# jsdjayanga/kmer-counter

Hardware: NVIDIA B200
Metric: k-mers counted/s at k=31 (higher is better)
Workload: dtype u64

## Files before the change

### kmer-counter_b200/csrc/kc_super.cu

```cuda
#include <math.h>
#include <stdlib.h>

#include "kc_internal.h"
#include "kc_super.cuh"

namespace kc {

namespace {

constexpr uint32_t kNoBin = 0xffffffffu;
constexpr int kSwThreads = 256;
constexpr int kSwMaxSeg = 18;
constexpr int kNb1Max = 1024;
constexpr int kRsBins = 2048;

template <uint32_t X> struct ILog2 { static constexpr uint32_t v = 1 + ILog2<(X >> 1)>::v; };
template <> struct ILog2<1> { static constexpr uint32_t v = 0; };

__host__ __device__ __forceinline__ uint32_t mmer_hash(uint32_t mm) {
    uint32_t h = mm * 0x9E3779B1u;
    h ^= h >> 15;
    h *= 0x85EBCA6Bu;
    return h;
}
__device__ __forceinline__ uint32_t bin_of_min(uint32_t mn, uint32_t n_bins) {
    return __umulhi(mn * 0xC2B2AE35u, n_bins);
}

struct SwScatterParams {
    ExtractParams ep;
    uint32_t m, w, nh, nh_stride, seg_len, segs_per_read, cmax, span;
    uint32_t h_off, bin_off, bits_off;
    uint32_t n_bins, bin_cap;
    uint64_t ovf_cap;
    uint32_t *cursor;
    uint8_t *bins;
    uint8_t *ovf;
    unsigned long long *sc;
};

template <int W, bool CANON>
__global__ void __launch_bounds__(kSwThreads) sw_scatter_kernel(SwScatterParams q) {
    const ExtractParams &p = q.ep;
    extern __shared__ __align__(128) uint8_t smem[];
    const uint32_t stage_bytes = p.stage_bytes;
    uint8_t *stage0 = smem;
    uint64_t *enc = reinterpret_cast<uint64_t *>(smem + p.enc_off);
    uint8_t *enc_b = reinterpret_cast<uint8_t *>(enc);
    const uint32_t enc_row = p.nw + 1;
    uint8_t *bad4 = smem + p.bad_off;
    uint8_t *flag = smem + p.flag_off;
    uint64_t *bars = reinterpret_cast<uint64_t *>(smem + p.bar_off);
    uint32_t *hh = reinterpret_cast<uint32_t *>(smem + q.h_off);
    uint32_t *bid = reinterpret_cast<uint32_t *>(smem + q.bin_off);
    uint32_t *seg_st = reinterpret_cast<uint32_t *>(smem + q.bits_off);
    uint32_t *seg_bd = seg_st + p.tile_reads * q.segs_per_read;
    __shared__ uint32_t s_nstart;
    const uint32_t tid = threadIdx.x, lane = tid & 31;

    if (tid == 0) {
        s_nstart = 0;
        mbar_init(&bars[0], 1);
        mbar_init(&bars[1], 1);
        mbar_fence_init();
    }
    for (uint32_t i = tid; i < p.tile_reads * enc_row; i += kSwThreads) enc[i] = 0;
    for (uint32_t i = tid; i < p.tile_reads; i += kSwThreads) flag[i] = 0;
    __syncthreads();

    auto tile_reads_of = [&](uint32_t t) -> uint32_t {
        uint64_t first = (uint64_t)t * p.tile_reads;
        uint64_t left = p.n_reads - first;
        return left < p.tile_reads ? (uint32_t)left : p.tile_reads;
    };
    auto issue_load = [&](uint32_t t, uint32_t s) {
        uint32_t bytes = tile_reads_of(t) * p.L;
        const uint8_t *src = p.reads + (uint64_t)t * p.tile_reads * p.L;
        uint8_t *dst = stage0 + s * stage_bytes;
        if ((bytes & 15u) == 0) {
            if (tid == 0) {
                asm volatile("fence.proxy.async.shared::cta;" ::: "memory");
                mbar_expect_tx(&bars[s], bytes);
                tma_load_1d(dst, src, bytes, &bars[s]);
            }
        } else {
            for (uint32_t i = tid; i < bytes; i += kSwThreads) dst[i] = src[i];
        }
    };

    uint32_t phase_bits = 0, stage = 0;
    unsigned long long invalid_local = 0, windows_local = 0, records_local = 0;
    const uint32_t mmask = q.m >= 16 ? 0xffffffffu : ((1u << (2 * q.m)) - 1u);
    const uint32_t mshift = 64 - 2 * q.m;
    const uint32_t ng = (q.nh + 7) >> 3;

    uint32_t tile = blockIdx.x;
    if (tile < p.n_tiles) issue_load(tile, 0);

    for (; tile < p.n_tiles; tile += gridDim.x) {
        const uint32_t next = tile + gridDim.x;
        if (next < p.n_tiles) issue_load(next, stage ^ 1);
        const uint32_t nreads = tile_reads_of(tile);
        if (((nreads * p.L) & 15u) == 0) {
            mbar_wait(&bars[stage], (phase_bits >> stage) & 1u);
            phase_bits ^= 1u << stage;
        } else {
            __syncthreads();
        }
        const uint8_t *src_tile = stage0 + stage * stage_bytes;

        encode_tile(p, src_tile, nreads, enc_b, bad4, flag);
        __syncthreads();
        if (tid == 0) s_nstart = 0;

        for (uint32_t g = tid; g < nreads * ng; g += kSwThreads) {
            const uint32_t r = g / ng, j0 = (g - r * ng) * 8;
            const uint32_t wi = j0 >> 5, sh = (j0 & 31u) * 2u;
            const uint64_t *e = enc + r * enc_row;
            const uint64_t a = wi <= p.nw ? e[wi] : 0ull;
            const uint64_t b = wi + 1 <= p.nw ? e[wi + 1] : 0ull;
            const uint64_t x = sh ? ((a << sh) | (b >> (64 - sh))) : a;
            uint32_t *row = hh + r * q.nh_stride + j0;
            if constexpr (CANON) {
#pragma unroll
                for (uint32_t i = 0; i < 8; i++) {
                    const uint32_t mm = (uint32_t)(x >> (mshift - 2 * i)) & mmask;
                    uint32_t r = __brev(mm);
                    r = ((r >> 1) & 0x55555555u) | ((r & 0x55555555u) << 1);
                    if (j0 + i < q.nh) row[i] = mmer_hash(min(mm, (r >> (32 - 2 * q.m)) ^ mmask));
                }
            } else {
#pragma unroll
                for (uint32_t i = 0; i < 8; i++)
                    if (j0 + i < q.nh) row[i] = mmer_hash((uint32_t)(x >> (mshift - 2 * i)) & mmask);
            }
        }
        __syncthreads();

        const uint32_t n_seg = nreads * q.segs_per_read;
        for (uint32_t sg = tid; sg < n_seg; sg += kSwThreads) {
            const uint32_t r = sg / q.segs_per_read;
            const uint32_t p0 = (sg - r * q.segs_per_read) * q.seg_len;
            if (p0 >= p.nk) { seg_st[sg] = 0; seg_bd[sg] = 0; continue; }
            const uint32_t s = min(q.seg_len, p.nk - p0);
            const uint32_t lb = p0 > 0 ? 1u : 0u;
            const uint32_t se = s + lb;
            const uint32_t *g = hh + r * q.nh_stride + p0 - lb;
            uint32_t S[kSwMaxSeg];
            S[kSwMaxSeg - 1] = 0xffffffffu;
#pragma unroll
            for (int i = kSwMaxSeg - 2; i >= 0; i--) {
                const uint32_t v = (uint32_t)i + 1 < se ? g[i] : 0xffffffffu;
                S[i] = min(v, S[i + 1]);
            }
            uint32_t core = 0xffffffffu;
            for (uint32_t t = se - 1; t < q.w; t++) core = min(core, g[t]);
            uint32_t pm = 0xffffffffu;
            const bool check = flag[r] != 0;
            uint32_t *brow = bid + r * p.nk + p0 - lb;
            uint32_t prev = kNoBin, stm = 0, bdm = 0;
#pragma unroll
            for (uint32_t i = 0; i < (uint32_t)kSwMaxSeg; i++) {
                if (i < se) {
                    const uint32_t mn = min(min(S[i], core), pm);
                    const bool valid = check ? kmer_window_valid(bad4 + r * p.nb4, p0 - lb + i, p.k) : true;
                    const uint32_t b = valid ? bin_of_min(mn, q.n_bins) : kNoBin;
                    if (i >= lb) {
                        if (!valid) invalid_local++;
                        brow[i] = b;
                        const uint32_t st = (valid && b != prev) ? 1u : 0u;
                        stm |= st << (i - lb);
                        bdm |= (st | (valid ? 0u : 1u)) << (i - lb);
                    }
                    prev = b;
                    if (i + 1 < se) pm = min(pm, g[q.w + i]);
                }
            }
            seg_st[sg] = stm;
            seg_bd[sg] = bdm;
        }
        __syncthreads();

        uint32_t *list = hh;
        for (uint32_t base = 0; base < n_seg; base += kSwThreads) {
            const uint32_t sg = base + tid;
            uint32_t stm = sg < n_seg ? seg_st[sg] : 0u;
            const uint32_t cnt = __popc(stm);
            uint32_t incl = cnt;
#pragma unroll
            for (int o = 1; o < 32; o <<= 1) {
                const uint32_t t = __shfl_up_sync(0xffffffffu, incl, o);
                if (lane >= (uint32_t)o) incl += t;
            }
            uint32_t off = 0;
            if (lane == 31 && incl) off = atomicAdd(&s_nstart, incl);
            off = __shfl_sync(0xffffffffu, off, 31) + incl - cnt;
            while (stm) {
                const uint32_t i = __ffs(stm) - 1;
                stm &= stm - 1;
                list[off++] = (sg << 5) | i;
            }
        }
        __syncthreads();
        const uint32_t n_start = s_nstart;
        for (uint32_t en = tid; en < n_start; en += kSwThreads) {
            const uint32_t ent = list[en];
            const uint32_t sg = ent >> 5, wi0 = ent & 31u;
            const uint32_t r = sg / q.segs_per_read, si = sg - r * q.segs_per_read;
            const uint32_t pos = si * q.seg_len + wi0;
            uint32_t end = p.nk;
            {
                uint32_t mk = seg_bd[sg] & ~(0xffffffffu >> (31 - wi0));
                uint32_t sj = si;
                while (mk == 0 && ++sj < q.segs_per_read) mk = seg_bd[r * q.segs_per_read + sj];
                if (mk) end = min(p.nk, sj * q.seg_len + (uint32_t)__ffs(mk) - 1);
            }
            const uint32_t len = end - pos;
            const uint32_t b = bid[r * p.nk + pos];
            const uint64_t *e = enc + r * enc_row;
            for (uint32_t q0 = 0; q0 < len; q0 += q.cmax) {
                const uint32_t idx = atomicAdd(&q.cursor[b], 1u);
                const uint32_t c = min(q.cmax, len - q0);
                const uint32_t wi = (pos + q0) >> 5, sh = ((pos + q0) & 31u) * 2u;
                uint64_t ew[2 * W + 1];
#pragma unroll
                for (int t = 0; t < 2 * W + 1; t++) ew[t] = wi + t <= p.nw ? e[wi + t] : 0ull;
                uint64_t rec[2 * W];
#pragma unroll
                for (int t = 0; t < 2 * W; t++) rec[t] = sh ? ((ew[t] << sh) | (ew[t + 1] >> (64 - sh))) : ew[t];
                const uint32_t nbases = q.span + c - 1;
#pragma unroll
                for (int t = 0; t < 2 * W; t++) {
                    const int keep = (int)nbases - 32 * t;
                    if (keep <= 0) rec[t] = 0;
                    else if (keep < 32) rec[t] &= ~0ull << (64 - 2 * keep);
                }
                rec[2 * W - 1] = (rec[2 * W - 1] & ~0xffull) | c;
                ulonglong2 *dst = nullptr;
                if (idx < q.bin_cap) {
                    dst = reinterpret_cast<ulonglong2 *>(q.bins) + ((uint64_t)b * q.bin_cap + idx) * W;
                } else {
                    const unsigned long long oi = atomicAdd(&q.sc[SW_OVF], 1ull);
                    if (oi < q.ovf_cap) dst = reinterpret_cast<ulonglong2 *>(q.ovf) + oi * W;
                    else atomicOr(&q.sc[SW_FAIL], 1ull);
                }
                if (dst) {
#pragma unroll
                    for (int t = 0; t < W; t++) dst[t] = make_ulonglong2(rec[2 * t], rec[2 * t + 1]);
                }
                windows_local += c;
                records_local++;
            }
        }
        for (uint32_t i = tid; i < nreads; i += kSwThreads) flag[i] = 0;
        __syncthreads();
        stage ^= 1;
    }
#pragma unroll
    for (int o = 16; o > 0; o >>= 1) {
        invalid_local += __shfl_xor_sync(0xffffffffu, invalid_local, o);
        windows_local += __shfl_xor_sync(0xffffffffu, windows_local, o);
        records_local += __shfl_xor_sync(0xffffffffu, records_local, o);
    }
    if (lane == 0) {
        if (invalid_local) atomicAdd(&q.sc[SW_INVALID], invalid_local);
        if (windows_local) atomicAdd(&q.sc[SW_WINDOWS], windows_local);
        if (records_local) atomicAdd(&q.sc[SW_RECORDS], records_local);
    }
}

template <int W> __device__ __forceinline__ bool key_all_ones(const Key<W> &k) {
    uint64_t a = ~0ull;
#pragma unroll
    for (int i = 0; i < W; i++) a &= k.w[i];
    return a == ~0ull;
}
template <int W> __device__ __forceinline__ bool key_any_word_ones(const Key<W> &k) {
    bool r = false;
#pragma unroll
    for (int i = 0; i < W; i++) r = r || (k.w[i] == ~0ull);
    return r;
}
template <int W> __device__ __forceinline__ void key_set_ones(Key<W> &k) {
#pragma unroll
    for (int i = 0; i < W; i++) k.w[i] = ~0ull;
}
__device__ __forceinline__ Key<1> slot_claim(Key<1> *slot, const Key<1> &k) {
    Key<1> o;
    o.w[0] = atomicCAS(reinterpret_cast<unsigned long long *>(slot), ~0ull, (unsigned long long)k.w[0]);
    return o;
}
__device__ __forceinline__ Key<2> slot_claim(Key<2> *slot, const Key<2> &k) {
    Key<2> o;
    const uint32_t a = smem_u32(slot);
    asm volatile(
        "{\n"
        ".reg .b128 c, n, o;\n"
        "mov.b128 c, {%3, %3};\n"
        "mov.b128 n, {%4, %5};\n"
        "atom.shared.cas.b128 o, [%2], c, n;\n"
        "mov.b128 {%0, %1}, o;\n"
        "}\n"
        : "=l"(o.w[0]), "=l"(o.w[1])
        : "r"(a), "l"(~0ull), "l"(k.w[0]), "l"(k.w[1])
        : "memory");
    return o;
}
template <int W> __device__ __forceinline__ uint32_t key_hash(const Key<W> &k) {
    uint32_t x = (uint32_t)k.w[0] ^ (uint32_t)(k.w[0] >> 29);
    if constexpr (W > 1) x ^= ((uint32_t)k.w[W - 1] ^ (uint32_t)(k.w[W - 1] >> 31)) * 0x85EBCA6Bu;
    return x * 0x9E3779B1u;
}
__device__ __forceinline__ uint32_t pass_hash(uint32_t h) { return (h ^ (h >> 15)) * 0x2C1B3C6Du; }

enum {
    SWP_UNIT = 0,
    SWP_DEDUP,
    SWP_SCAN,
    SWP_OPEN,
    SWP_INSERT,
    SWP_DRAIN,
    SWP_ROUND_END,
    SWP_EMIT,
    SWP_PHASES,
    SWP_QUEUED = SWP_PHASES,
    SWP_DRAIN_PROBES,
    SWP_WARPS,
    SWP_TOTAL,
    SWP_SLOTS
};
#ifdef KC_SW_PROFILE
__device__ unsigned long long g_sw_prof[SWP_SLOTS];
#define SWP_DECL                                                                                      \
    __shared__ unsigned long long s_prof[THREADS / 32][SWP_SLOTS];                                    \
    if (lane == 0)                                                                                    \
        for (int i_ = 0; i_ < SWP_SLOTS; i_++) s_prof[warp][i_] = 0;                                  \
    const long long swp_t0 = clock64();                                                               \
    long long swp_t = swp_t0
#define SWP_MARK(ph)                                                                                  \
    do {                                                                                              \
        const long long t_ = clock64();                                                               \
        if (lane == 0) s_prof[warp][ph] += (unsigned long long)(t_ - swp_t);                          \
        swp_t = t_;                                                                                   \
    } while (0)
#define SWP_ADD(c, v) atomicAdd(&s_prof[warp][c], (unsigned long long)(v))
#define SWP_ADD_ACTIVE(c)                                                                             \
    do {                                                                                              \
        const uint32_t am_ = __activemask();                                                          \
        if (lane == (uint32_t)__ffs(am_) - 1) SWP_ADD(c, __popc(am_));                                \
    } while (0)
#define SWP_FLUSH()                                                                                   \
    do {                                                                                              \
        __syncwarp();                                                                                 \
        if (lane == 0) {                                                                              \
            s_prof[warp][SWP_WARPS] = 1;                                                              \
            s_prof[warp][SWP_TOTAL] = (unsigned long long)(clock64() - swp_t0);                       \
            for (int i_ = 0; i_ < SWP_SLOTS; i_++) atomicAdd(&g_sw_prof[i_], s_prof[warp][i_]);       \
        }                                                                                             \
    } while (0)
#else
#define SWP_DECL do {} while (0)
#define SWP_MARK(ph) do {} while (0)
#define SWP_ADD(c, v) do {} while (0)
#define SWP_ADD_ACTIVE(c) do {} while (0)
#define SWP_FLUSH() do {} while (0)
#endif

struct SwCountParams {
    uint32_t n_src;
    const uint32_t *src_cursor[8];
    const uint8_t *src_bins[8];
    const unsigned long long *src_sc[8];
    uint32_t bin_begin;
    const uint8_t *ovf;
    uint32_t n_bins, bin_cap, ovf_slice;
    uint64_t ovf_cap;
    uint64_t last_mask;
    uint64_t *d_keys;
    uint32_t *d_counts;
    uint64_t d_cap;
    uint32_t *hist1;
    int shift1, nb1;
    int add_phantom;
    unsigned long long *sc;
};

template <int W> struct SwCountCfg {
    static constexpr int THREADS = 512, TSLOTS = 4096, RPT = W == 1 ? 2 : 1;
};

template <int W, int THREADS, int TSLOTS, int RPT, bool CANON>
__global__ void __launch_bounds__(THREADS) sw_count_kernel(SwCountParams p) {
    constexpr int RB = THREADS * RPT;
    extern __shared__ __align__(16) uint8_t cs_smem[];
    Key<W> *tk = reinterpret_cast<Key<W> *>(cs_smem);
    ulonglong2 *recs = reinterpret_cast<ulonglong2 *>(tk + TSLOTS);
    uint32_t *tc = reinterpret_cast<uint32_t *>(recs + RB * W);
    uint32_t *s_start = tc + TSLOTS;
    uint32_t *s_hist = s_start + THREADS;
    constexpr int kQueue = RPT > 1 ? 64 : 96;
    Key<W> *queue = reinterpret_cast<Key<W> *>(s_hist + kNb1Max);
    uint32_t *queue_m = reinterpret_cast<uint32_t *>(queue + (THREADS / 32) * kQueue);
    constexpr bool DEDUP = (W == 1);
    constexpr int RT = DEDUP ? RB : 1;
    ulonglong2 *rt_keys = reinterpret_cast<ulonglong2 *>(queue_m + (THREADS / 32) * kQueue);
    uint32_t *rt_mult = reinterpret_cast<uint32_t *>(rt_keys + RT);
    uint32_t *rec_mult = rt_mult + RT;
    __shared__ uint32_t s_unit, s_m, s_ones, s_abort;
    __shared__ unsigned long long s_base;
    __shared__ uint32_t s_warp[THREADS / 32];
// ... 1268 lines not shown
    pl.w = pl.span - pl.m + 1;
    pl.nh = pl.nk + pl.w - 1;
    pl.nh_stride = (pl.nh + 8) | 1u;
    pl.seg_len = pl.w - 1 < (uint32_t)kSwMaxSeg - 1 ? pl.w - 1 : (uint32_t)kSwMaxSeg - 1;
    pl.segs_per_read = (pl.nk + pl.seg_len - 1) / pl.seg_len;
    pl.seg_len = (pl.nk + pl.segs_per_read - 1) / pl.segs_per_read;
}
}

bool super_plan(uint32_t k, uint32_t L, uint32_t flags, uint64_t max_windows, uint32_t occ_per_bin, SuperPlan *out,
                double record_headroom, uint64_t distinct_hint, bool ext_e) {
    if (k == 0 || k > 64 || L < k || L > 4096) return false;
    if (flags & kPlanCanonical) flags |= kPlanStrict;
    const bool strict = (flags & kPlanStrict) != 0;
    SuperPlan pl{};
    pl.flags = flags & (kPlanStrict | kPlanCanonical);
    pl.W = (int)((k + 31) / 32);
    pl.k = k;
    pl.L = L;
    const uint32_t mm = k % 32;
    const bool masked = strict ? (mm != 0) : (mm >= 1 && mm <= 28);
    pl.span = masked ? k : 32u * pl.W;
    pl.last_mask = masked ? (~0ull << (64 - 2 * mm)) : ~0ull;
    if (pl.span < 22) return false;
    pl.nk = L - k + 1;
    pl.cmax = 32u * pl.W - 3;
    if (max_windows == 0) max_windows = 1;
    if (occ_per_bin == 0) {
        occ_per_bin = 8192;
        if (distinct_hint && distinct_hint < max_windows) {
            const double per_key = (double)max_windows / (double)distinct_hint;
            const double occ = 2200.0 * per_key;
            if (occ < 8192.0) occ_per_bin = occ < 1024.0 ? 1024u : ((uint32_t)occ + 255u) & ~255u;
        }
    }
    uint64_t nb = (max_windows + occ_per_bin - 1) / occ_per_bin;
    if (nb < 8) nb = 8;
    if (nb > (1ull << 24)) nb = 1ull << 24;
    pl.n_bins = (uint32_t)nb;
    ExtractParams ep;
    if (!extract_plan(nullptr, 16, L, k, pl.flags, nullptr, &ep, kS1TileBytes)) return false;
    set_minimizer(pl, 12);
    if (s1_smem(pl, ep).total > kS1MaxSmem) return false;
    while (pl.m < 16 && pl.m + 8 < pl.span && (1ull << (2 * pl.m)) < 192ull * pl.n_bins) {
        SuperPlan longer = pl;
        set_minimizer(longer, pl.m + 1);
        if (s1_smem(longer, ep).total > kS1MaxSmem) break;
        pl = longer;
    }
    const double rho = 2.0 / (pl.w + 1) + 1.2 / pl.nk + 1.0 / pl.cmax * 0.25;
    const double est_total = (double)max_windows * rho;
    const double per_bin = est_total / (double)pl.n_bins;
    pl.bin_cap = (uint32_t)(per_bin * (1.0 + 90.0 / sqrt((double)occ_per_bin))) + 64;
    pl.bin_cap = (pl.bin_cap + 3) & ~3u;
    pl.ovf_cap = (uint64_t)(est_total * 0.6) + 8192;
    if (pl.ovf_cap < max_windows / 16) pl.ovf_cap = max_windows / 16;
    pl.ovf_slice = 4096;
    const uint64_t d_base = distinct_hint && distinct_hint < max_windows ? distinct_hint + distinct_hint / 8 + 4096 : max_windows;
    pl.d_cap = d_base + (uint64_t)((double)d_base * record_headroom) + (record_headroom > 0 ? 8192 : 0);
    if (pl.d_cap > (1ull << 32) - 2) pl.d_cap = (1ull << 32) - 2;
    if (pl.d_cap < 1024) pl.d_cap = 1024;
    pl.fin_cap = pl.d_cap > (uint64_t)kSuperMaxSub * (kFinCapSmall * 7 / 10) ? kFinCapLarge : kFinCapSmall;
    pl.sub_target = pl.fin_cap * 7 / 10;
    if (const char *v = getenv("KC_SW_SUB_TARGET")) {
        const int t = atoi(v);
        if (t > 0) pl.sub_target = (uint32_t)t;
    }
    const int sig = pl.W == 1 ? (masked ? (int)(2 * mm) : 64) : 64;
    pl.b1 = sig < 10 ? sig : 10;
    plan_layout(pl, ext_e);
    *out = pl;
    return true;
}

static void plan_layout(SuperPlan &pl, bool ext_e) {
    uint64_t o = 0;
    auto take = [&](uint64_t bytes) { uint64_t r = o; o += round512(bytes); return r; };
    const uint64_t rec_bytes = 16ull * pl.W;
    pl.off_cursor = take((uint64_t)pl.n_bins * 4);
    pl.off_hist1 = take((kNb1Max + 8) * 4);
    pl.off_hist2 = take((uint64_t)(2 * kSuperMaxSub + 8) * 4);
    pl.off_base1 = take((kNb1Max + 8) * 4);
    pl.off_cur1 = take((kNb1Max + 8) * 4);
    pl.off_base2 = take((uint64_t)(kSuperMaxSub + 8) * 4);
    pl.off_cur2 = take((uint64_t)(kSuperMaxSub + 8) * 4);
    pl.off_mout = take((uint64_t)(kSuperMaxSub + 8) * 4);
    pl.off_off = take((uint64_t)(kSuperMaxSub + 8) * 4);
    pl.off_plan = take(sizeof(SuperPlanDev));
    pl.off_x = take(sizeof(XDev));
    pl.off_sc = take(SW_COUNT * 8);
    pl.off_h2m = take((uint64_t)(kSuperMaxSub + 8) * 4);
    pl.off_big = take((uint64_t)(kSuperMaxSub + 8) * 4);
    pl.off_bigoff = take((uint64_t)(kSuperMaxSub + 8) * 4);
    pl.off_bins = take((uint64_t)pl.n_bins * pl.bin_cap * rec_bytes);
    pl.off_ovf = take(pl.ovf_cap * rec_bytes);
    pl.off_dk = take(pl.d_cap * 8 * pl.W + 64);
    pl.off_dc = take(pl.d_cap * 4 + 64);
    pl.ext_e = ext_e;
    pl.ext_ek = nullptr;
    pl.ext_ec = nullptr;
    pl.off_ek = pl.off_ec = o;
    if (!ext_e) {
        pl.off_ek = take(pl.d_cap * 8 * pl.W + 64);
        pl.off_ec = take(pl.d_cap * 4 + 64);
    }
    pl.ws_bytes = o;
}

bool place_plan(uint32_t k, bool strict, uint64_t n_records, SuperPlan *out) {
    if (k == 0 || k > 128 || n_records == 0 || n_records > (1ull << 32) - 2) return false;
    SuperPlan pl{};
    pl.W = (int)((k + 31) / 32);
    pl.k = k;
    const uint32_t mm = k % 32;
    const bool masked = strict ? (mm != 0) : (mm >= 1 && mm <= 28);
    pl.span = masked ? k : 32u * pl.W;
    pl.last_mask = masked ? (~0ull << (64 - 2 * mm)) : ~0ull;
    pl.n_bins = 8;
    pl.d_cap = n_records < 1024 ? 1024 : n_records;
    pl.fin_cap = pl.W >= 3 && n_records <= (uint64_t)kSuperMaxSub * (kFinCapWide * 7 / 10) ? kFinCapWide : kFinCapSmall;
    pl.sub_target = pl.fin_cap * 7 / 10;
    if (const char *v = getenv("KC_SW_SUB_TARGET")) {
        const int t = atoi(v);
        if (t > 0) pl.sub_target = (uint32_t)t;
    }
    const int sig = pl.W == 1 ? (masked ? (int)(2 * mm) : 64) : 64;
    pl.b1 = sig < 10 ? sig : 10;
    plan_layout(pl, false);
    *out = pl;
    return true;
}

namespace {
template <class T> T *at(void *ws, uint64_t off) { return reinterpret_cast<T *>(static_cast<uint8_t *>(ws) + off); }
uint64_t *ek_of(const SuperPlan &pl, void *ws) { return pl.ext_e ? pl.ext_ek : at<uint64_t>(ws, pl.off_ek); }
uint32_t *ec_of(const SuperPlan &pl, void *ws) { return pl.ext_e ? pl.ext_ec : at<uint32_t>(ws, pl.off_ec); }
}

cudaError_t super_reset(const SuperPlan &pl, void *ws, unsigned long long *d_sc, cudaStream_t s) {
    cudaError_t e;
    if ((e = cudaMemsetAsync(ws, 0, pl.off_base1, s)) != cudaSuccess) return e;
    return cudaMemsetAsync(d_sc, 0, SW_COUNT * 8, s);
}

template <int W>
static cudaError_t super_scatter_w(const SuperPlan &pl, const void *d_reads, uint64_t n_reads, void *ws,
                                   unsigned long long *d_sc, int n_sms, cudaStream_t s) {
    SwScatterParams q{};
    if (!extract_plan(d_reads, n_reads, pl.L, pl.k, pl.flags, &d_sc[SW_INVALID], &q.ep, kS1TileBytes))
        return cudaErrorInvalidValue;
    if (q.ep.n_tiles == 0) return cudaSuccess;
    q.m = pl.m; q.w = pl.w; q.nh = pl.nh; q.nh_stride = pl.nh_stride;
    q.seg_len = pl.seg_len; q.segs_per_read = pl.segs_per_read; q.cmax = pl.cmax; q.span = pl.span;
    const S1Smem lay = s1_smem(pl, q.ep);
    q.h_off = lay.h_off;
    q.bin_off = lay.bin_off;
    q.bits_off = lay.bits_off;
    const uint32_t smem = lay.total;
    if (smem > kS1MaxSmem) return cudaErrorInvalidValue;
    q.n_bins = pl.n_bins; q.bin_cap = pl.bin_cap; q.ovf_cap = pl.ovf_cap;
    q.cursor = at<uint32_t>(ws, pl.off_cursor);
    q.bins = at<uint8_t>(ws, pl.off_bins);
    q.ovf = at<uint8_t>(ws, pl.off_ovf);
    q.sc = d_sc;
    auto kern = (pl.flags & kPlanCanonical) ? sw_scatter_kernel<W, true> : sw_scatter_kernel<W, false>;
    cudaError_t e = cudaFuncSetAttribute(kern, cudaFuncAttributeMaxDynamicSharedMemorySize, (int)smem);
    if (e != cudaSuccess) return e;
    int per_sm = 1;
    cudaOccupancyMaxActiveBlocksPerMultiprocessor(&per_sm, kern, kSwThreads, smem);
    per_sm = per_sm < 1 ? 1 : (per_sm > 6 ? 6 : per_sm);
    uint32_t grid = (uint32_t)n_sms * per_sm;
    if (grid > q.ep.n_tiles) grid = q.ep.n_tiles;
    kern<<<grid, kSwThreads, smem, s>>>(q);
    return cudaGetLastError();
}

cudaError_t super_scatter(const SuperPlan &pl, const void *d_reads, uint64_t n_reads, void *ws,
                          unsigned long long *d_sc, int n_sms, cudaStream_t s) {
    if (pl.W == 1) return super_scatter_w<1>(pl, d_reads, n_reads, ws, d_sc, n_sms, s);
    if (pl.W == 2) return super_scatter_w<2>(pl, d_reads, n_reads, ws, d_sc, n_sms, s);
    return cudaErrorInvalidValue;
}

template <int W, bool CANON>
static cudaError_t launch_count(const SwCountParams &cp, int n_sms, cudaStream_t s) {
    constexpr uint32_t THREADS = SwCountCfg<W>::THREADS, TSLOTS = SwCountCfg<W>::TSLOTS, RPT = SwCountCfg<W>::RPT;
    const uint32_t RB = THREADS * RPT, RT = W == 1 ? RB : 1;
    const uint32_t smem = TSLOTS * (8 * W + 4) + RB * 16 * W + THREADS * 4 + kNb1Max * 4 +
                          (THREADS / 32) * (RPT > 1 ? 64 : 96) * (8 * W + 4) + RT * 20 + RB * 4 + 64;
    auto kern = sw_count_kernel<W, THREADS, TSLOTS, RPT, CANON>;
    cudaError_t e = cudaFuncSetAttribute(kern, cudaFuncAttributeMaxDynamicSharedMemorySize, (int)smem);
    if (e != cudaSuccess) return e;
    int per_sm = 1;
    cudaOccupancyMaxActiveBlocksPerMultiprocessor(&per_sm, kern, THREADS, smem);
    if (per_sm < 1) per_sm = 1;
    kern<<<(uint32_t)n_sms * per_sm, THREADS, smem, s>>>(cp);
    return cudaGetLastError();
}

template <int W>
static cudaError_t super_count_bins_w(const SuperPlan &pl, bool add_phantom, void *ws, unsigned long long *d_sc, int n_sms,
                                      cudaStream_t s, void *const *peer_ws = nullptr, uint32_t rank = 0,
                                      uint32_t n_ranks = 1) {
    SwCountParams cp{};
    const uint32_t n_src = peer_ws ? n_ranks : 1u;
    cp.n_src = n_src;
    for (uint32_t i = 0; i < n_src; i++) {
        void *w = peer_ws ? peer_ws[i] : ws;
        cp.src_cursor[i] = at<uint32_t>(w, pl.off_cursor);
        cp.src_bins[i] = at<uint8_t>(w, pl.off_bins);
        cp.src_sc[i] = peer_ws ? at<unsigned long long>(w, pl.off_sc) : d_sc;
    }
    cp.bin_begin = peer_ws ? (uint32_t)((uint64_t)pl.n_bins * rank / n_ranks) : 0u;
    cp.n_bins = peer_ws ? (uint32_t)((uint64_t)pl.n_bins * (rank + 1) / n_ranks) - cp.bin_begin : pl.n_bins;
    cp.ovf = at<uint8_t>(ws, pl.off_ovf);
    cp.bin_cap = pl.bin_cap; cp.ovf_slice = pl.ovf_slice; cp.ovf_cap = pl.ovf_cap;
    cp.last_mask = pl.last_mask;
    cp.d_keys = at<uint64_t>(ws, pl.off_dk); cp.d_counts = at<uint32_t>(ws, pl.off_dc); cp.d_cap = pl.d_cap;
    cp.hist1 = at<uint32_t>(ws, pl.off_hist1); cp.shift1 = 64 - pl.b1; cp.nb1 = 1 << pl.b1;
    cp.add_phantom = add_phantom ? 1 : 0;
    cp.sc = d_sc;
    return (pl.flags & kPlanCanonical) ? launch_count<W, true>(cp, n_sms, s) : launch_count<W, false>(cp, n_sms, s);
}

cudaError_t super_count_bins(const SuperPlan &pl, bool add_phantom, void *ws, unsigned long long *d_sc, int n_sms,
                             cudaStream_t s, void *const *peer_ws, uint32_t rank, uint32_t n_ranks) {
    if (peer_ws && (n_ranks == 0 || n_ranks > 8 || rank >= n_ranks)) return cudaErrorInvalidValue;
    if (pl.W == 1) return super_count_bins_w<1>(pl, add_phantom, ws, d_sc, n_sms, s, peer_ws, rank, n_ranks);
    if (pl.W == 2) return super_count_bins_w<2>(pl, add_phantom, ws, d_sc, n_sms, s, peer_ws, rank, n_ranks);
    return cudaErrorInvalidValue;
}

template <int W>
static cudaError_t super_place_w(const SuperPlan &pl, void *ws, unsigned long long *d_sc, int n_sms, cudaStream_t s,
                                 cudaEvent_t *evs) {
    cudaError_t e;
    uint64_t *dk = at<uint64_t>(ws, pl.off_dk), *ek = ek_of(pl, ws);
    uint32_t *dc = at<uint32_t>(ws, pl.off_dc), *ec = ec_of(pl, ws);
    if (!ek || !ec) return cudaErrorInvalidValue;
    uint32_t *hist1 = at<uint32_t>(ws, pl.off_hist1), *base1 = at<uint32_t>(ws, pl.off_base1),
             *cur1 = at<uint32_t>(ws, pl.off_cur1), *hist2 = at<uint32_t>(ws, pl.off_hist2),
             *base2 = at<uint32_t>(ws, pl.off_base2), *cur2 = at<uint32_t>(ws, pl.off_cur2);
    SuperPlanDev *plan = at<SuperPlanDev>(ws, pl.off_plan);
    const int sig = pl.W == 1 ? 64 - (int)__builtin_ctzll(pl.last_mask ? pl.last_mask : 1) : 64;
    sw_plan_kernel<<<1, 1024, 0, s>>>(hist1, pl.b1, pl.d_cap, pl.sub_target, sig, base1, cur1, plan, d_sc);
    const uint32_t rs_smem = RsCfg<W>::TILE * (8 * W + 4) + 3 * kRsBinsPadded * 4;
    auto k1 = rec_scatter_kernel<W, 1>;
    auto k2 = rec_scatter_kernel<W, 2>;
    if ((e = cudaFuncSetAttribute(k1, cudaFuncAttributeMaxDynamicSharedMemorySize, (int)rs_smem)) != cudaSuccess) return e;
    if ((e = cudaFuncSetAttribute(k2, cudaFuncAttributeMaxDynamicSharedMemorySize, (int)rs_smem)) != cudaSuccess) return e;
    int per_sm = 1;
    cudaOccupancyMaxActiveBlocksPerMultiprocessor(&per_sm, k1, kRsThreads, rs_smem);
    if (per_sm < 1) per_sm = 1;
    const uint32_t grid = (uint32_t)n_sms * per_sm;
    k1<<<grid, kRsThreads, rs_smem, s>>>(dk, dc, ek, ec, plan, pl.b1, &d_sc[SW_D], pl.d_cap, cur1, nullptr);
    if ((e = cudaGetLastError()) != cudaSuccess) return e;
    if (evs) cudaEventRecord(evs[0], s);
    rec_hist2_kernel<W><<<(uint32_t)n_sms * 8, 256, 0, s>>>(ek, plan, hist2);
    sw_scan_kernel<<<(kSuperMaxSub + kScanTile - 1) / kScanTile, 1024, 0, s>>>(hist2, &plan->n_sub, 0, base2, cur2, nullptr);
    if ((e = cudaGetLastError()) != cudaSuccess) return e;
    if (evs) cudaEventRecord(evs[1], s);
    k2<<<grid, kRsThreads, rs_smem, s>>>(ek, ec, dk, dc, plan, pl.b1, &d_sc[SW_D], pl.d_cap, cur2, nullptr);
    if ((e = cudaGetLastError()) != cudaSuccess) return e;
    if (evs) cudaEventRecord(evs[2], s);
    return cudaSuccess;
}

cudaError_t super_place(const SuperPlan &pl, void *ws, unsigned long long *d_sc, int n_sms, cudaStream_t s, cudaEvent_t *evs) {
    if (pl.W == 1) return super_place_w<1>(pl, ws, d_sc, n_sms, s, evs);
    if (pl.W == 2) return super_place_w<2>(pl, ws, d_sc, n_sms, s, evs);
    if (pl.W == 3) return super_place_w<3>(pl, ws, d_sc, n_sms, s, evs);
    if (pl.W == 4) return super_place_w<4>(pl, ws, d_sc, n_sms, s, evs);
    return cudaErrorInvalidValue;
}

cudaError_t place_init(const SuperPlan &pl, void *ws, unsigned long long *d_sc, uint64_t n, int n_sms, cudaStream_t s) {
    cudaError_t e;
    if (n > pl.d_cap) return cudaErrorInvalidValue;
    if ((e = cudaMemsetAsync(ws, 0, pl.off_base1, s)) != cudaSuccess) return e;
    const uint64_t *dk = at<uint64_t>(ws, pl.off_dk);
    uint32_t *dc = at<uint32_t>(ws, pl.off_dc), *hist1 = at<uint32_t>(ws, pl.off_hist1);
    const uint32_t grid = (uint32_t)n_sms * 8;
    const int shift1 = 64 - pl.b1;
    switch (pl.W) {
        case 1: place_init_kernel<1><<<grid, 256, 0, s>>>(dk, dc, n, shift1, hist1, d_sc); break;
        case 2: place_init_kernel<2><<<grid, 256, 0, s>>>(dk, dc, n, shift1, hist1, d_sc); break;
        case 3: place_init_kernel<3><<<grid, 256, 0, s>>>(dk, dc, n, shift1, hist1, d_sc); break;
        case 4: place_init_kernel<4><<<grid, 256, 0, s>>>(dk, dc, n, shift1, hist1, d_sc); break;
        default: return cudaErrorInvalidValue;
    }
    return cudaGetLastError();
}

uint64_t *place_keys(const SuperPlan &pl, void *ws) { return at<uint64_t>(ws, pl.off_dk); }

cudaError_t place_fix_zero(int W, const uint64_t *run_keys, uint32_t *run_counts, const unsigned long long *d_n_invalid,
                           cudaStream_t s) {
    switch (W) {
        case 1: place_fix_zero_kernel<1><<<1, 1, 0, s>>>(run_keys, run_counts, d_n_invalid); break;
        case 2: place_fix_zero_kernel<2><<<1, 1, 0, s>>>(run_keys, run_counts, d_n_invalid); break;
        case 3: place_fix_zero_kernel<3><<<1, 1, 0, s>>>(run_keys, run_counts, d_n_invalid); break;
        case 4: place_fix_zero_kernel<4><<<1, 1, 0, s>>>(run_keys, run_counts, d_n_invalid); break;
        default: return cudaErrorInvalidValue;
    }
    return cudaGetLastError();
}
// ... 52 lines not shown
    if (!dup || (pl.fin_cap != kFinCapSmall && pl.fin_cap != kFinCapWide)) return cudaErrorInvalidValue;
    if (pl.fin_cap == kFinCapWide) {
        if (pl.W == 3) return super_finish_w<3, true, 256, kFinCapWide>(pl, ws, d_sc, out_keys, out_counts, n_sms, s);
        if (pl.W == 4) return super_finish_w<4, true, 256, kFinCapWide>(pl, ws, d_sc, out_keys, out_counts, n_sms, s);
    } else {
        if (pl.W == 3) return super_finish_w<3, true, 512, kFinCapSmall>(pl, ws, d_sc, out_keys, out_counts, n_sms, s);
        if (pl.W == 4) return super_finish_w<4, true, 512, kFinCapSmall>(pl, ws, d_sc, out_keys, out_counts, n_sms, s);
    }
    return cudaErrorInvalidValue;
}

cudaError_t super_big_gather(const SuperPlan &pl, void *ws, uint64_t *tk, uint32_t *tc, int n_sms, cudaStream_t s) {
    SuperPlanDev *plan = at<SuperPlanDev>(ws, pl.off_plan);
    uint32_t *big = at<uint32_t>(ws, pl.off_big), *bigoff = at<uint32_t>(ws, pl.off_bigoff), *base2 = at<uint32_t>(ws, pl.off_base2);
    sw_scan_kernel<<<(kSuperMaxSub + kScanTile - 1) / kScanTile, 1024, 0, s>>>(big, &plan->n_sub, 0, bigoff, nullptr, nullptr);
    const uint64_t *dk = at<uint64_t>(ws, pl.off_dk);
    const uint32_t *dc = at<uint32_t>(ws, pl.off_dc);
    if (pl.W == 1) big_gather_kernel<1><<<(uint32_t)n_sms * 8, 256, 0, s>>>(dk, dc, base2, big, bigoff, plan, tk, tc);
    else if (pl.W == 2) big_gather_kernel<2><<<(uint32_t)n_sms * 8, 256, 0, s>>>(dk, dc, base2, big, bigoff, plan, tk, tc);
    else if (pl.W == 3) big_gather_kernel<3><<<(uint32_t)n_sms * 8, 256, 0, s>>>(dk, dc, base2, big, bigoff, plan, tk, tc);
    else big_gather_kernel<4><<<(uint32_t)n_sms * 8, 256, 0, s>>>(dk, dc, base2, big, bigoff, plan, tk, tc);
    return cudaGetLastError();
}

cudaError_t super_big_place(const SuperPlan &pl, bool dup, void *ws, unsigned long long *d_sc, const uint64_t *sk,
                            const uint32_t *sc_counts, uint64_t *out_keys, uint32_t *out_counts, int n_sms, cudaStream_t s) {
    const SuperPlanDev *plan = at<SuperPlanDev>(ws, pl.off_plan);
    const uint32_t *big = at<uint32_t>(ws, pl.off_big), *bigoff = at<uint32_t>(ws, pl.off_bigoff), *base2 = at<uint32_t>(ws, pl.off_base2);
    uint32_t *m_out = at<uint32_t>(ws, pl.off_mout);
    const uint32_t grid = (uint32_t)n_sms * 8;
    if (pl.W == 1) {
        if (dup) big_place_kernel<1, true><<<grid, 256, 0, s>>>(sk, sc_counts, base2, big, bigoff, plan, out_keys, out_counts, m_out, d_sc);
        else big_place_kernel<1, false><<<grid, 256, 0, s>>>(sk, sc_counts, base2, big, bigoff, plan, out_keys, out_counts, m_out, d_sc);
    } else if (pl.W == 2) {
        if (dup) big_place_kernel<2, true><<<grid, 256, 0, s>>>(sk, sc_counts, base2, big, bigoff, plan, out_keys, out_counts, m_out, d_sc);
        else big_place_kernel<2, false><<<grid, 256, 0, s>>>(sk, sc_counts, base2, big, bigoff, plan, out_keys, out_counts, m_out, d_sc);
    } else if (pl.W == 3 && dup) {
        big_place_kernel<3, true><<<grid, 256, 0, s>>>(sk, sc_counts, base2, big, bigoff, plan, out_keys, out_counts, m_out, d_sc);
    } else if (pl.W == 4 && dup) {
        big_place_kernel<4, true><<<grid, 256, 0, s>>>(sk, sc_counts, base2, big, bigoff, plan, out_keys, out_counts, m_out, d_sc);
    } else {
        return cudaErrorInvalidValue;
    }
    return cudaGetLastError();
}

cudaError_t super_fold_offsets(const SuperPlan &pl, void *ws, unsigned long long *d_sc, cudaStream_t s) {
    SuperPlanDev *plan = at<SuperPlanDev>(ws, pl.off_plan);
    sw_scan_kernel<<<(kSuperMaxSub + kScanTile - 1) / kScanTile, 1024, 0, s>>>(
        at<uint32_t>(ws, pl.off_mout), &plan->n_sub, 0, at<uint32_t>(ws, pl.off_off), nullptr, &d_sc[SW_OUT]);
    return cudaGetLastError();
}

cudaError_t super_gather(const SuperPlan &pl, void *ws, const uint64_t *tmp_keys, const uint32_t *tmp_counts,
                         uint64_t *out_keys, uint32_t *out_counts, int n_sms, cudaStream_t s) {
    const SuperPlanDev *plan = at<SuperPlanDev>(ws, pl.off_plan);
    const uint32_t *src = at<uint32_t>(ws, pl.off_base2), *off = at<uint32_t>(ws, pl.off_off);
    if (pl.W == 1) sw_gather_kernel<1><<<(uint32_t)n_sms * 8, 256, 0, s>>>(tmp_keys, tmp_counts, src, off, plan, out_keys, out_counts);
    else if (pl.W == 2) sw_gather_kernel<2><<<(uint32_t)n_sms * 8, 256, 0, s>>>(tmp_keys, tmp_counts, src, off, plan, out_keys, out_counts);
    else if (pl.W == 3) sw_gather_kernel<3><<<(uint32_t)n_sms * 8, 256, 0, s>>>(tmp_keys, tmp_counts, src, off, plan, out_keys, out_counts);
    else sw_gather_kernel<4><<<(uint32_t)n_sms * 8, 256, 0, s>>>(tmp_keys, tmp_counts, src, off, plan, out_keys, out_counts);
    return cudaGetLastError();
}

void super_use_large_finish(SuperPlan *pl) { pl->fin_cap = kFinCapLarge; }

template <int W>
static cudaError_t super_x_local_w(const SuperPlan &pl, void *ws, unsigned long long *d_sc, const uint32_t *d_all_hist,
                                   uint32_t rank, uint32_t n_ranks, bool keep_ranges, void *const *peer_ws, int n_sms,
                                   cudaStream_t s) {
    cudaError_t e;
    if (pl.ext_e) return cudaErrorInvalidValue;
    uint64_t *dk = at<uint64_t>(ws, pl.off_dk), *ek = at<uint64_t>(ws, pl.off_ek);
    uint32_t *dc = at<uint32_t>(ws, pl.off_dc), *ec = at<uint32_t>(ws, pl.off_ec);
    SuperPlanDev *plan = at<SuperPlanDev>(ws, pl.off_plan);
    const int sig = pl.W == 1 ? 64 - (int)__builtin_ctzll(pl.last_mask ? pl.last_mask : 1) : 64;
    XScalars xs{};
    for (uint32_t i = 0; i < n_ranks; i++) xs.sc[i] = peer_ws ? at<unsigned long long>(peer_ws[i], pl.off_sc) : d_sc;
    x_plan_kernel<<<1, 1024, 0, s>>>(d_all_hist, rank, n_ranks, keep_ranges ? 1 : 0, pl.d_cap, pl.sub_target,
                                     pl.fin_cap == kFinCapLarge ? 1 : 0, sig, at<uint32_t>(ws, pl.off_base1),
                                     at<uint32_t>(ws, pl.off_cur1), plan, at<XDev>(ws, pl.off_x), d_sc, xs);
    const uint32_t rs_smem = RsCfg<W>::TILE * (8 * W + 4) + 3 * kRsBinsPadded * 4;
    auto k1 = rec_scatter_kernel<W, 1>;
    if ((e = cudaFuncSetAttribute(k1, cudaFuncAttributeMaxDynamicSharedMemorySize, (int)rs_smem)) != cudaSuccess) return e;
    int per_sm = 1;
    cudaOccupancyMaxActiveBlocksPerMultiprocessor(&per_sm, k1, kRsThreads, rs_smem);
    if (per_sm < 1) per_sm = 1;
    k1<<<(uint32_t)n_sms * per_sm, kRsThreads, rs_smem, s>>>(dk, dc, ek, ec, plan, pl.b1, &d_sc[SW_D], pl.d_cap,
                                                            at<uint32_t>(ws, pl.off_cur1), nullptr);
    rec_hist2_kernel<W><<<(uint32_t)n_sms * 8, 256, 0, s>>>(ek, plan, at<uint32_t>(ws, pl.off_hist2));
    return cudaGetLastError();
}

cudaError_t super_x_local(const SuperPlan &pl, void *ws, unsigned long long *d_sc, const uint32_t *d_all_hist,
                          uint32_t rank, uint32_t n_ranks, bool keep_ranges, void *const *peer_ws, int n_sms, cudaStream_t s) {
    if (pl.b1 != kXB1 || n_ranks == 0 || n_ranks > 8 || rank >= n_ranks) return cudaErrorInvalidValue;
    if (pl.W == 1) return super_x_local_w<1>(pl, ws, d_sc, d_all_hist, rank, n_ranks, keep_ranges, peer_ws, n_sms, s);
    if (pl.W == 2) return super_x_local_w<2>(pl, ws, d_sc, d_all_hist, rank, n_ranks, keep_ranges, peer_ws, n_sms, s);
    return cudaErrorInvalidValue;
}

template <int W>
static cudaError_t super_x_pull_w(const SuperPlan &pl, void *ws, unsigned long long *d_sc, void *const *peer_ws,
                                  uint32_t rank, uint32_t n_ranks, int n_sms, cudaStream_t s) {
    cudaError_t e;
    SuperPlanDev *plan = at<SuperPlanDev>(ws, pl.off_plan);
    XDev *x = at<XDev>(ws, pl.off_x);
    XPeers peers{};
    for (uint32_t i = 0; i < n_ranks; i++) {
        peers.keys[i] = at<uint64_t>(peer_ws[i], pl.off_ek);
        peers.counts[i] = at<uint32_t>(peer_ws[i], pl.off_ec);
        peers.hist2[i] = at<uint32_t>(peer_ws[i], pl.off_hist2);
    }
    uint32_t *h2m = at<uint32_t>(ws, pl.off_h2m), *base2 = at<uint32_t>(ws, pl.off_base2), *cur2 = at<uint32_t>(ws, pl.off_cur2);
    x_merge_hist_kernel<<<(uint32_t)n_sms * 4, 256, 0, s>>>(peers, n_ranks, plan, h2m);
    sw_scan_kernel<<<(kSuperMaxSub + kScanTile - 1) / kScanTile, 1024, 0, s>>>(h2m, &plan->n_sub, 0, base2, cur2, nullptr);
    const uint32_t rs_smem = RsCfg<W>::TILE * (8 * W + 4) + 3 * kRsBinsPadded * 4;
    auto k2 = rec_scatter_kernel<W, 2>;
    if ((e = cudaFuncSetAttribute(k2, cudaFuncAttributeMaxDynamicSharedMemorySize, (int)rs_smem)) != cudaSuccess) return e;
    int per_sm = 1;
    cudaOccupancyMaxActiveBlocksPerMultiprocessor(&per_sm, k2, kRsThreads, rs_smem);
    if (per_sm < 1) per_sm = 1;
    for (uint32_t j = 1; j <= n_ranks; j++) {
        const uint32_t i = (rank + j) % n_ranks;
        k2<<<(uint32_t)n_sms * per_sm, kRsThreads, rs_smem, s>>>(peers.keys[i], peers.counts[i], at<uint64_t>(ws, pl.off_dk),
                                                                at<uint32_t>(ws, pl.off_dc), plan, pl.b1, &d_sc[SW_D],
                                                                pl.d_cap, cur2, &x->src_range[i][0]);
    }
    return cudaGetLastError();
}

cudaError_t super_x_pull(const SuperPlan &pl, void *ws, unsigned long long *d_sc, void *const *peer_ws, uint32_t rank,
                         uint32_t n_ranks, int n_sms, cudaStream_t s) {
    if (n_ranks == 0 || n_ranks > 8 || rank >= n_ranks) return cudaErrorInvalidValue;
    if (pl.W == 1) return super_x_pull_w<1>(pl, ws, d_sc, peer_ws, rank, n_ranks, n_sms, s);
    if (pl.W == 2) return super_x_pull_w<2>(pl, ws, d_sc, peer_ws, rank, n_ranks, n_sms, s);
    return cudaErrorInvalidValue;
}

uint32_t *super_hist1(const SuperPlan &pl, void *ws) { return at<uint32_t>(ws, pl.off_hist1); }
const SuperXInfo *super_x_info(const SuperPlan &pl, void *ws) { return at<XDev>(ws, pl.off_x); }

}

#ifdef KC_SW_PROFILE
extern "C" int kc_sw_profile_read(unsigned long long *out, int reset) {
    cudaError_t e = cudaMemcpyFromSymbol(out, kc::g_sw_prof, sizeof(kc::g_sw_prof));
    if (e == cudaSuccess && reset) {
        static const unsigned long long zero[kc::SWP_SLOTS] = {};
        e = cudaMemcpyToSymbol(kc::g_sw_prof, zero, sizeof(zero));
    }
    return e == cudaSuccess ? 0 : -1;
}
#endif
```

Baseline: 60.44 billion.

## Streamline stage-1 scatter with magic division, funnel shifts and bitmask segment logic

Replaces integer divisions by ng and segs_per_read with precomputed multiply-high magic division. Extracts m-mers with 32-bit funnel shifts and drops the per-element nh bounds check. Restructures the minimizer segment loop so invalid windows are computed once as a bitmask and start/boundary masks come from bitwise ops instead of per-element branches. Also adds compile-time-gated per-phase clock profiling. Dropping the nh guard means writes past nh into row padding must be safe.

Measured after the change: 63.87 billion, median of 6. 1.06x the previous value.

```diff
diff --git a/kmer-counter_b200/csrc/kc_super.cu b/kmer-counter_b200/csrc/kc_super.cu
--- a/kmer-counter_b200/csrc/kc_super.cu
+++ b/kmer-counter_b200/csrc/kc_super.cu
@@ -8,7 +8,6 @@
 
 namespace {
 
-constexpr uint32_t kNoBin = 0xffffffffu;
 constexpr int kSwThreads = 256;
 constexpr int kSwMaxSeg = 18;
 constexpr int kNb1Max = 1024;
@@ -27,9 +26,58 @@
     return __umulhi(mn * 0xC2B2AE35u, n_bins);
 }
 
+enum {
+    S1P_LOAD = 0,
+    S1P_ENCODE,
+    S1P_HASH,
+    S1P_MIN,
+    S1P_STARTS,
+    S1P_RECORDS,
+    S1P_BARRIER,
+    S1P_PHASES,
+    S1P_WARPS = S1P_PHASES,
+    S1P_TOTAL,
+    S1P_SLOTS
+};
+#ifdef KC_SW_PROFILE
+__device__ unsigned long long g_s1_prof[S1P_SLOTS];
+#define S1P_DECL                                                                                      \
+    __shared__ unsigned long long s1_prof[kSwThreads / 32][S1P_SLOTS];                               \
+    if (lane == 0)                                                                                    \
+        for (int i_ = 0; i_ < S1P_SLOTS; i_++) s1_prof[tid >> 5][i_] = 0;                            \
+    const long long s1p_t0 = clock64();                                                               \
+    long long s1p_t = s1p_t0
+#define S1P_MARK(ph)                                                                                  \
+    do {                                                                                              \
+        const long long t_ = clock64();                                                               \
+        if (lane == 0) s1_prof[tid >> 5][ph] += (unsigned long long)(t_ - s1p_t);                     \
+        s1p_t = t_;                                                                                   \
+    } while (0)
+#define S1P_FLUSH()                                                                                   \
+    do {                                                                                              \
+        __syncwarp();                                                                                 \
+        if (lane == 0) {                                                                              \
+            s1_prof[tid >> 5][S1P_WARPS] = 1;                                                         \
+            s1_prof[tid >> 5][S1P_TOTAL] = (unsigned long long)(clock64() - s1p_t0);                  \
+            for (int i_ = 0; i_ < S1P_SLOTS; i_++) atomicAdd(&g_s1_prof[i_], s1_prof[tid >> 5][i_]);  \
+        }                                                                                             \
+    } while (0)
+#else
+#define S1P_DECL do {} while (0)
+#define S1P_MARK(ph) do {} while (0)
+#define S1P_FLUSH() do {} while (0)
+#endif
+
+__device__ __forceinline__ uint32_t div_magic(uint32_t x, uint32_t d, uint32_t magic) {
+    if (d == 1) return x;
+    uint32_t r = __umulhi(x, magic);
+    return r * d > x ? r - 1 : r;
+}
+
 struct SwScatterParams {
     ExtractParams ep;
     uint32_t m, w, nh, nh_stride, seg_len, segs_per_read, cmax, span;
+    uint32_t ng, ng_magic, segs_magic;
     uint32_t h_off, bin_off, bits_off;
     uint32_t n_bins, bin_cap;
     uint64_t ovf_cap;
@@ -57,6 +105,7 @@
     uint32_t *seg_bd = seg_st + p.tile_reads * q.segs_per_read;
     __shared__ uint32_t s_nstart;
     const uint32_t tid = threadIdx.x, lane = tid & 31;
+    S1P_DECL;
 
     if (tid == 0) {
         s_nstart = 0;
@@ -91,8 +140,8 @@
     uint32_t phase_bits = 0, stage = 0;
     unsigned long long invalid_local = 0, windows_local = 0, records_local = 0;
     const uint32_t mmask = q.m >= 16 ? 0xffffffffu : ((1u << (2 * q.m)) - 1u);
-    const uint32_t mshift = 64 - 2 * q.m;
-    const uint32_t ng = (q.nh + 7) >> 3;
+    const uint32_t mshift = 32 - 2 * q.m;
+    const uint32_t ng = q.ng;
 
     uint32_t tile = blockIdx.x;
     if (tile < p.n_tiles) issue_load(tile, 0);
@@ -108,38 +157,44 @@
             __syncthreads();
         }
         const uint8_t *src_tile = stage0 + stage * stage_bytes;
+        S1P_MARK(S1P_LOAD);
 
         encode_tile(p, src_tile, nreads, enc_b, bad4, flag);
-        __syncthreads();
+        S1P_MARK(S1P_ENCODE);
+        __syncthreads();
+        S1P_MARK(S1P_BARRIER);
         if (tid == 0) s_nstart = 0;
 
         for (uint32_t g = tid; g < nreads * ng; g += kSwThreads) {
-            const uint32_t r = g / ng, j0 = (g - r * ng) * 8;
+            const uint32_t r = div_magic(g, ng, q.ng_magic), j0 = (g - r * ng) * 8;
             const uint32_t wi = j0 >> 5, sh = (j0 & 31u) * 2u;
             const uint64_t *e = enc + r * enc_row;
             const uint64_t a = wi <= p.nw ? e[wi] : 0ull;
             const uint64_t b = wi + 1 <= p.nw ? e[wi + 1] : 0ull;
             const uint64_t x = sh ? ((a << sh) | (b >> (64 - sh))) : a;
+            const uint32_t xh = (uint32_t)(x >> 32), xl = (uint32_t)x;
             uint32_t *row = hh + r * q.nh_stride + j0;
             if constexpr (CANON) {
 #pragma unroll
                 for (uint32_t i = 0; i < 8; i++) {
-                    const uint32_t mm = (uint32_t)(x >> (mshift - 2 * i)) & mmask;
+                    const uint32_t mm = __funnelshift_l(xl, xh, 2 * i) >> mshift;
                     uint32_t r = __brev(mm);
                     r = ((r >> 1) & 0x55555555u) | ((r & 0x55555555u) << 1);
-                    if (j0 + i < q.nh) row[i] = mmer_hash(min(mm, (r >> (32 - 2 * q.m)) ^ mmask));
+                    row[i] = mmer_hash(min(mm, (r >> (32 - 2 * q.m)) ^ mmask));
                 }
             } else {
 #pragma unroll
                 for (uint32_t i = 0; i < 8; i++)
-                    if (j0 + i < q.nh) row[i] = mmer_hash((uint32_t)(x >> (mshift - 2 * i)) & mmask);
-            }
-        }
-        __syncthreads();
+                    row[i] = mmer_hash(__funnelshift_l(xl, xh, 2 * i) >> mshift);
+            }
+        }
+        S1P_MARK(S1P_HASH);
+        __syncthreads();
+        S1P_MARK(S1P_BARRIER);
 
         const uint32_t n_seg = nreads * q.segs_per_read;
         for (uint32_t sg = tid; sg < n_seg; sg += kSwThreads) {
-            const uint32_t r = sg / q.segs_per_read;
+            const uint32_t r = div_magic(sg, q.segs_per_read, q.segs_magic);
             const uint32_t p0 = (sg - r * q.segs_per_read) * q.seg_len;
             if (p0 >= p.nk) { seg_st[sg] = 0; seg_bd[sg] = 0; continue; }
             const uint32_t s = min(q.seg_len, p.nk - p0);
@@ -155,31 +210,28 @@
             }
             uint32_t core = 0xffffffffu;
             for (uint32_t t = se - 1; t < q.w; t++) core = min(core, g[t]);
-            uint32_t pm = 0xffffffffu;
-            const bool check = flag[r] != 0;
+            uint32_t inv = 0;
+            if (flag[r] != 0)
+                for (uint32_t i = 0; i < se; i++)
+                    if (!kmer_window_valid(bad4 + r * p.nb4, p0 - lb + i, p.k)) inv |= 1u << i;
+            uint32_t pm = 0xffffffffu, prev = 0, eq = 0;
             uint32_t *brow = bid + r * p.nk + p0 - lb;
-            uint32_t prev = kNoBin, stm = 0, bdm = 0;
 #pragma unroll
             for (uint32_t i = 0; i < (uint32_t)kSwMaxSeg; i++) {
-                if (i < se) {
-                    const uint32_t mn = min(min(S[i], core), pm);
-                    const bool valid = check ? kmer_window_valid(bad4 + r * p.nb4, p0 - lb + i, p.k) : true;
-                    const uint32_t b = valid ? bin_of_min(mn, q.n_bins) : kNoBin;
-                    if (i >= lb) {
-                        if (!valid) invalid_local++;
-                        brow[i] = b;
-                        const uint32_t st = (valid && b != prev) ? 1u : 0u;
-                        stm |= st << (i - lb);
-                        bdm |= (st | (valid ? 0u : 1u)) << (i - lb);
-                    }
-                    prev = b;
-                    if (i + 1 < se) pm = min(pm, g[q.w + i]);
-                }
-            }
-            seg_st[sg] = stm;
-            seg_bd[sg] = bdm;
-        }
-        __syncthreads();
+                const uint32_t b = bin_of_min(min(min(S[i], core), pm), q.n_bins);
+                if (i >= lb && i < se) brow[i] = b;
+                if (i > 0 && b == prev) eq |= 1u << i;
+                prev = b;
+                pm = min(pm, i + 1 < se ? g[q.w + i] : 0xffffffffu);
+            }
+            const uint32_t st = ~inv & (~eq | (inv << 1)) & ((1u << se) - 1u);
+            seg_st[sg] = st >> lb;
+            seg_bd[sg] = (st | inv) >> lb;
+            invalid_local += __popc(inv >> lb);
+        }
+        S1P_MARK(S1P_MIN);
+        __syncthreads();
+        S1P_MARK(S1P_BARRIER);
 
         uint32_t *list = hh;
         for (uint32_t base = 0; base < n_seg; base += kSwThreads) {
@@ -201,12 +253,14 @@
                 list[off++] = (sg << 5) | i;
             }
         }
-        __syncthreads();
+        S1P_MARK(S1P_STARTS);
+        __syncthreads();
+        S1P_MARK(S1P_BARRIER);
         const uint32_t n_start = s_nstart;
         for (uint32_t en = tid; en < n_start; en += kSwThreads) {
             const uint32_t ent = list[en];
             const uint32_t sg = ent >> 5, wi0 = ent & 31u;
-            const uint32_t r = sg / q.segs_per_read, si = sg - r * q.segs_per_read;
+            const uint32_t r = div_magic(sg, q.segs_per_read, q.segs_magic), si = sg - r * q.segs_per_read;
             const uint32_t pos = si * q.seg_len + wi0;
             uint32_t end = p.nk;
             {
@@ -253,9 +307,12 @@
             }
         }
         for (uint32_t i = tid; i < nreads; i += kSwThreads) flag[i] = 0;
-        __syncthreads();
+        S1P_MARK(S1P_RECORDS);
+        __syncthreads();
+        S1P_MARK(S1P_BARRIER);
         stage ^= 1;
     }
+    S1P_FLUSH();
 #pragma unroll
     for (int o = 16; o > 0; o >>= 1) {
         invalid_local += __shfl_xor_sync(0xffffffffu, invalid_local, o);
@@ -1830,6 +1887,9 @@
     if (q.ep.n_tiles == 0) return cudaSuccess;
     q.m = pl.m; q.w = pl.w; q.nh = pl.nh; q.nh_stride = pl.nh_stride;
     q.seg_len = pl.seg_len; q.segs_per_read = pl.segs_per_read; q.cmax = pl.cmax; q.span = pl.span;
+    q.ng = (pl.nh + 7) >> 3;
+    q.ng_magic = (uint32_t)((1ull << 32) / q.ng + 1);
+    q.segs_magic = (uint32_t)((1ull << 32) / q.segs_per_read + 1);
     const S1Smem lay = s1_smem(pl, q.ep);
     q.h_off = lay.h_off;
     q.bin_off = lay.bin_off;
@@ -2188,4 +2248,12 @@
     }
     return e == cudaSuccess ? 0 : -1;
 }
+extern "C" int kc_s1_profile_read(unsigned long long *out, int reset) {
+    cudaError_t e = cudaMemcpyFromSymbol(out, kc::g_s1_prof, sizeof(kc::g_s1_prof));
+    if (e == cudaSuccess && reset) {
+        static const unsigned long long zero[kc::S1P_SLOTS] = {};
+        e = cudaMemcpyToSymbol(kc::g_s1_prof, zero, sizeof(zero));
+    }
+    return e == cudaSuccess ? 0 : -1;
+}
 #endif
```
